# NVIDIA/nvalchemi-toolkit-ops

Measured on AMD Instinct MI355X. Metric: atom-steps/sec (nlist+D3+PME) on 100k-atom PBC box, higher is better.
Workload: dtype f64 (PME) + f32 (D3)

## Files before the change

### nvalchemi-toolkit-ops_amd/csrc/d3.hip

```cpp
#include <type_traits>
#include <mutex>

#include "common.h"
#include "binsort.h"

#ifdef MI_D3_IEEE
#define D3_RCP(x) (1.0f / (x))
#define D3_SQRT(x) sqrtf(x)
#else
#define D3_RCP(x) __builtin_amdgcn_rcpf(x)
#define D3_SQRT(x) __builtin_amdgcn_sqrtf(x)
#endif

namespace {

struct D3Dev {
  const float* rcov;
  const float* r4r2;
  const float4* tab;
  int nz;
  float a1, a2, s6, s8, k1, k3, s5_on, s5_off, inv_w;
  float4* crec;
  const float* crc;
  int* cflag;
// ... 17 lines not shown
  f.pad_code = S;
  return f;
}
__device__ __forceinline__ float d3_crec_encode(float d, int id, const D3CRec& f, bool* bad) {
  *bad = !(fabsf(d) < 256.0f);
  unsigned u = (unsigned)__float_as_int(d * f.down);
  if (f.mbit) u = (u + 1u) & ~1u;
  u |= ((unsigned)id << f.eshift) & f.emask;
  u |= ((unsigned)id >> f.eb) & f.mbit;
  return __int_as_float((int)u);
}
__device__ __forceinline__ int d3_crec_id(float w, const D3CRec& f) {
  const unsigned u = (unsigned)__float_as_int(w);
  return (int)(((u & f.emask) >> f.eshift) | ((u & f.mbit) << f.eb));
}
__device__ __forceinline__ float d3_crec_value(float w, const D3CRec& f) { return __int_as_float((int)((unsigned)__float_as_int(w) & f.clear)); }

struct D3Species;
__device__ __forceinline__ int d3_species_count(const D3Species* info);
struct D3ZeroSpec { const float* r0ab; float irs6, irs8, beta; };
struct D3ZeroPair { float i6, i8, bR; };
__device__ __forceinline__ D3ZeroPair d3_zero_pair(const D3ZeroSpec& Z, int zi, int zj, int nz) {
  const float R0 = Z.r0ab[(size_t)zi * nz + zj];
  const bool ok = R0 > 0.0f;
  D3ZeroPair p;
  p.i6 = ok ? Z.irs6 / R0 : 0.0f; p.i8 = ok ? Z.irs8 / R0 : 0.0f; p.bR = ok ? Z.beta * R0 : 0.0f;
  return p;
}
__device__ __forceinline__ float d3_zero_w(const D3ZeroSpec& Z, int zi, int zj, int nz, int pq) {
  if (Z.r0ab == nullptr || pq > 2) return 0.0f;
  const D3ZeroPair p = d3_zero_pair(Z, zi, zj, nz);
  return pq == 0 ? p.i6 : (pq == 1 ? p.i8 : p.bR);
}
struct D3Tables { const float* c6ab; const float* cnref; int nz; const D3Species* info; float4* tab; int first_block; D3ZeroSpec zero; };
__device__ __forceinline__ void d3_pack_tables_body(const float* __restrict__ c6ab, const float* __restrict__ cnref, int nz, const D3Species* __restrict__ info,
                                      float4* __restrict__ tab, long long vblock, const D3ZeroSpec& zero) {
  if (d3_species_count(info) <= 16) return;
  const long long t = vblock * blockDim.x + threadIdx.x;
  const long long total = (long long)nz * nz * 25;
  if (t >= total) return;
  const int pq = (int)(t % 25), p = pq / 5, q = pq % 5;
  const long long zz = t / 25;
  const int zj = (int)(zz % nz), zi = (int)(zz / nz);
  const float c6 = c6ab[t];
  const float ci = cnref[t];
  const float cj = cnref[(((long long)zj * nz + zi) * 5 + q) * 5 + p];
  tab[t] = make_float4(c6, ci, cj, d3_zero_w(zero, zi, zj, nz, pq));
}

template <class T> struct PairGeom { float r, rinv, rx, ry, rz; bool ok; };
struct Int3 { int a, b, c; };

#define D3_SORT_MIN_ATOMS 2048
#define D3_SORT_PER_BIN 16.0
template <class T> __device__ __forceinline__ T d3_code_pack(int place, int z);
template <> __device__ __forceinline__ float d3_code_pack<float>(int place, int z) { return __int_as_float((place << 7) | z); }
template <> __device__ __forceinline__ double d3_code_pack<double>(int place, int z) { return (double)(((long long)place << 7) | z); }
__device__ __forceinline__ int d3_code_of(float w) { return __float_as_int(w); }
__device__ __forceinline__ int d3_code_of(double w) { return (int)(long long)w; }

struct D3Grid { int cpd[3]; int off; };
template <class T>
__global__ void d3_sort_setup_kernel(const T* __restrict__ cell, int B, int N, float rc_est, D3Grid* __restrict__ grid, long long cap) {
  for (int s0 = 0; s0 < B; s0 += blockDim.x) {
    const int sidx = s0 + threadIdx.x;
    if (sidx < B) {
      T c[9], ci[9];
      for (int k = 0; k < 9; ++k) c[k] = cell[9 * (size_t)sidx + k];
      inverse3(c, ci);
      const double det = (double)c[0] * ((double)c[4] * c[8] - (double)c[5] * c[7]) - (double)c[1] * ((double)c[3] * c[8] - (double)c[5] * c[6]) +
// ... 39 lines not shown
    const int sidx = batch_idx ? batch_idx[i] : 0;
    const D3Grid G = grid[sidx];
    T c[9], ci[9];
    for (int k = 0; k < 9; ++k) c[k] = cell[9 * (size_t)sidx + k];
    inverse3(c, ci);
    const T x = pos[3 * (size_t)i], y = pos[3 * (size_t)i + 1], z = pos[3 * (size_t)i + 2];
    for (int d = 0; d < 3; ++d) {
      T f = x * ci[d] + y * ci[3 + d] + z * ci[6 + d];
      f = f - floor(f);
      const int q = (int)(f * (T)G.cpd[d]);
      n[d] = G.cpd[d];
      g[d] = q < 0 ? 0 : (q >= n[d] ? n[d] - 1 : q);
    }
    gs = sidx;
    key = G.off + (g[2] * n[1] + g[1]) * n[0] + g[0];
  }
  if (count) {
    if (in) keys[i] = key;
    bs_wave_add<false>(count, key, in);
  }
  const int nx_ = __shfl_down(g[0], 1, MI_WAVE), ny_ = __shfl_down(g[1], 1, MI_WAVE), nz_ = __shfl_down(g[2], 1, MI_WAVE), ns_ = __shfl_down(gs, 1, MI_WAVE);
  auto far = [](int a, int b, int m) { int d = a > b ? a - b : b - a; d = d < m - d ? d : m - d; return d > 1; };
  const bool pair = in && i + 1 < N && (threadIdx.x & (MI_WAVE - 1)) != MI_WAVE - 1;
  const bool bad = pair && (ns_ != gs || far(g[0], nx_, n[0]) || far(g[1], ny_, n[1]) || far(g[2], nz_, n[2]));
  const unsigned long long m = __ballot(bad);
  if (m && (threadIdx.x & (MI_WAVE - 1)) == 0) atomicAdd(incoherent, (int)__popcll(m));
}

#define D3_VERIFY_CHUNK 512
struct D3Guard {
  unsigned long long* slots; float K; const void* cell; int n_cell; const int* batch_idx;
  const int* nm; const int* nsh; const unsigned* words; const int* hdr_flag; int* flag; int M; int stride, phase; int atom_blocks;
};
template <class T>
__global__ void d3_pack_atoms_kernel(const T* __restrict__ pos, const int* __restrict__ numbers, int N, const float* __restrict__ rcov,
                                     const float* __restrict__ r4r2, const int* __restrict__ smap, int nz,
                                     typename Vec4<T>::type* __restrict__ apos, float4* __restrict__ aaux, float* __restrict__ forces,
                                     float* __restrict__ cn, float* __restrict__ dEdCN, float* __restrict__ e_atom, double* __restrict__ v_atom,
                                     const int* __restrict__ inv, typename Vec4<T>::type* __restrict__ apos_s, float4* __restrict__ aaux_s,
                                     typename Vec4<T>::type* __restrict__ acn, D3Guard G, D3Tables TB, float4* __restrict__ crec) {
  if ((int)blockIdx.x >= TB.first_block) {
    d3_pack_tables_body(TB.c6ab, TB.cnref, TB.nz, TB.info, TB.tab, (long long)blockIdx.x - TB.first_block, TB.zero);
    return;
  }
  if ((int)blockIdx.x >= G.atom_blocks) {
    const int lane = threadIdx.x & (MI_WAVE - 1);
    const int w = ((int)blockIdx.x - G.atom_blocks) * (blockDim.x / MI_WAVE) + threadIdx.x / MI_WAVE;
    if (w == 0 && lane == 0 && *G.hdr_flag != 0) *G.flag = 1;
    if (G.stride <= 0) return;
    const int chunks = 1, all_chunks = (G.M + D3_VERIFY_CHUNK - 1) / D3_VERIFY_CHUNK;
    const long long blk = w / chunks;
    const long long row = blk * G.stride + (long long)(((unsigned long long)G.phase + mi_mix64(0x51ull + (unsigned long long)blk)) % (unsigned long long)G.stride);
    if (row >= N) return;
    const int pick = G.stride == 1 ? -1 : (int)(mi_mix64(0x77ull + (unsigned long long)row * 1315423911ull + (unsigned long long)G.phase / (unsigned long long)G.stride) % (unsigned long long)all_chunks);
    const int t_beg = pick < 0 ? 0 : pick * D3_VERIFY_CHUNK, t_end = pick < 0 ? G.M : (t_beg + D3_VERIFY_CHUNK < G.M ? t_beg + D3_VERIFY_CHUNK : G.M);
    bool bad = false;
#pragma unroll 4
    for (int t = t_beg + lane; t < t_end; t += MI_WAVE) {
      const long long e = row * G.M + t;
      const int j = G.nm[e];
      const Int3 sh = reinterpret_cast<const Int3*>(G.nsh)[e];
      const unsigned cx = (unsigned)(sh.a + 1), cy = (unsigned)(sh.b + 1), cz = (unsigned)(sh.c + 1);
      const bool entry = (unsigned)j < (unsigned)N;
      const unsigned want = entry ? ((unsigned)j | ((cx & 3u) << 26) | ((cy & 3u) << 28) | (cz << 30)) : 0xffffffffu;
      bad |= G.words[e] != want || (entry && (cx > 2u || cy > 2u || cz > 2u));
    }
    if (bad) *G.flag = 1;
    return;
  }
  const int k = blockIdx.x * blockDim.x + threadIdx.x;
  if (G.slots) {
    unsigned long long h = 0;
    if (k < N) {
      const int a = inv ? inv[k] : k;
      h = mi_cn_atom_hash<T>(a, G.batch_idx ? G.batch_idx[a] : 0, pos[3 * (size_t)a], pos[3 * (size_t)a + 1], pos[3 * (size_t)a + 2],
                             mi_cn_rk(numbers[a], nz, rcov, G.K));
    }
    if (k < G.n_cell) h += mi_cn_cell_hash<T>(k, reinterpret_cast<const T*>(G.cell)[k]);
    if (k == 0) h += mi_cn_scale_hash(G.K);
    mi_cn_slot_add(G.slots, k / MI_WAVE, h);
  }
  if (k >= N) return;
  const int i = inv ? inv[k] : k;
  forces[3 * (size_t)i] = forces[3 * (size_t)i + 1] = forces[3 * (size_t)i + 2] = 0.0f;
  cn[i] = dEdCN[i] = e_atom[i] = 0.0f;
  if (v_atom)
    for (int k = 0; k < 9; ++k) v_atom[9 * (size_t)i + k] = 0.0;
  const int z = numbers[i];
  const bool real = z > 0 && z < nz;
  typename Vec4<T>::type r;
  r.x = pos[3 * (size_t)i]; r.y = pos[3 * (size_t)i + 1]; r.z = pos[3 * (size_t)i + 2];
  r.w = real ? (T)rcov[z] : (T)-1;
  apos[i] = r;
  const int sj = real ? smap[z] : -1;
  const float4 ax = make_float4(0.0f, real ? r4r2[z] : 0.0f, __int_as_float((z << 8) | (sj & 0xff)), 0.0f);
  aaux[i] = ax;
  if (crec) {
    const D3CRec f = d3_crec_format(d3_species_count(TB.info));
    bool bad;
    if (f.on) crec[k] = make_float4((float)r.x, (float)r.y, (float)r.z, d3_crec_encode(0.0f, sj >= 0 ? sj : f.pad_code, f, &bad));
  }
  if (inv) {
    apos_s[k] = r;
    aaux_s[k] = ax;
    r.w = d3_code_pack<T>(k, real ? z : 0);
    acn[i] = r;
  }
}

template <class T, class V4>
__device__ __forceinline__ PairGeom<T> d3_geom(const V4& pj, T pix, T piy, T piz, const Int3& sh, const T* __restrict__ cm, bool periodic) {
  PairGeom<T> g;
  T dx = pj.x - pix, dy = pj.y - piy, dz = pj.z - piz;
  if (periodic) {
    const T fs[3] = {(T)sh.a, (T)sh.b, (T)sh.c};
    T cart[3];
    const bool ortho = cm[1] == T(0) && cm[2] == T(0) && cm[3] == T(0) && cm[5] == T(0) && cm[6] == T(0) && cm[7] == T(0);
    if (ortho) { cart[0] = fs[0] * cm[0]; cart[1] = fs[1] * cm[4]; cart[2] = fs[2] * cm[8]; }
    else rowvec_mat3(fs, cm, cart);
    dx = dx + cart[0]; dy = dy + cart[1]; dz = dz + cart[2];
  }
  g.rx = (float)dx; g.ry = (float)dy; g.rz = (float)dz;
  const float r2 = g.rx * g.rx + g.ry * g.ry + g.rz * g.rz;
  g.ok = !(r2 < 1e-24f);
#ifdef MI_D3_IEEE
  g.r = sqrtf(g.ok ? r2 : 1.0f);
  const float rinv = 1.0f / g.r;
#else
  const float rinv = __builtin_amdgcn_rsqf(g.ok ? r2 : 1.0f);
  g.r = r2 * rinv;
#endif
// ... 232 lines not shown
    return;
  }
  const bool from_companion = *comp_flag == 0;
  for (int vb = blockIdx.x; vb < n_blocks; vb += gridDim.x) {
    if (from_companion) d3_cn_body<T, false, true, false, true>(D3_CN_ARGS, vb);
    else d3_cn_body<T, false, true, false, false>(D3_CN_ARGS, vb);
    __syncthreads();
  }
}
#undef D3_CN_ARGS
#undef D3_CN_PARAMS

__device__ __forceinline__ void d3_s5(float r, float on, float off, float inv_w, float& sw, float& dsw) {
  if (off <= on) { sw = 1.0f; dsw = 0.0f; return; }
  if (r <= on) { sw = 1.0f; dsw = 0.0f; return; }
  if (r >= off) { sw = 0.0f; dsw = 0.0f; return; }
  const float t = (r - on) * inv_w, t2 = t * t, t3 = t2 * t, t4 = t3 * t, t5 = t4 * t;
  sw = 1.0f - (10.0f * t3 - 15.0f * t4 + 6.0f * t5);
  dsw = (-30.0f * t2 + 60.0f * t3 - 30.0f * t4) * inv_w;
}

#define D3_SMAX 16

struct D3Species { int S; int factorized; int pad[2]; };
__device__ __forceinline__ int d3_species_count(const D3Species* info) { return info->S; }
#define D3_FROW 44

__global__ void d3_mark_species_kernel(const int* __restrict__ numbers, int N, int nz, int* __restrict__ present) {
  const int i = blockIdx.x * blockDim.x + threadIdx.x;
  if (i >= N) return;
  const int z = numbers[i];
  if (z > 0 && z < nz) present[z] = 1;
}
__global__ void d3_compact_species_kernel(const int* __restrict__ present, const float* __restrict__ c6ab, const float* __restrict__ cnref, int nz,
                                          int* __restrict__ smap, D3Species* __restrict__ info, float4* __restrict__ ctab,
                                          float* __restrict__ ftab, float* __restrict__ fcr, float k3, const float* __restrict__ r4r2,
                                          float a1, float a2, const float* __restrict__ rcov, float* __restrict__ crc, D3ZeroSpec zero) {
  __shared__ int zlist[D3_SMAX];
  __shared__ int count;
  __shared__ int fact_ok;
  if (threadIdx.x == 0) {
    fact_ok = 1;
    int S = 0;
    for (int z = 0; z < nz; ++z) {
      if (z > 0 && present[z]) { smap[z] = S < D3_SMAX ? S : -1; if (S < D3_SMAX) zlist[S] = z; ++S; }
      else smap[z] = -1;
    }
    count = S;
    info->S = S;
  }
  __syncthreads();
  const int S = count;
  if (S > D3_SMAX) { if (threadIdx.x == 0) info->factorized = 0; return; }
  if (threadIdx.x < 16) crc[threadIdx.x] = (int)threadIdx.x < S ? rcov[zlist[threadIdx.x]] : -1.0f;
  for (int k = threadIdx.x; k < S * S * 25; k += blockDim.x) {
    const int pq = k % 25, p = pq / 5, q = pq % 5, sj = (k / 25) % S, si = k / (25 * S);
    const int zi = zlist[si], zj = zlist[sj];
    const size_t a = ((size_t)zi * nz + zj) * 25 + pq, b = (((size_t)zj * nz + zi) * 5 + q) * 5 + p;
    ctab[k] = make_float4(c6ab[a], cnref[a], cnref[b], d3_zero_w(zero, zi, zj, nz, pq));
    ftab[((size_t)si * S + sj) * D3_FROW + p * 8 + q] = c6ab[a];
    const size_t dii = ((size_t)zi * nz + zi) * 25 + p * 6, djj = ((size_t)zj * nz + zj) * 25 + q * 6;
    const bool valid = c6ab[a] != 0.0f, rect = (c6ab[dii] != 0.0f) && (c6ab[djj] != 0.0f);
    const bool same = __float_as_int(cnref[a]) == __float_as_int(cnref[dii]) && __float_as_int(cnref[b]) == __float_as_int(cnref[djj]);
    if (valid != rect || (valid && !same)) fact_ok = 0;
  }
  for (int k = threadIdx.x; k < S * S * 5; k += blockDim.x) {
    float* row = ftab + (size_t)(k / 5) * D3_FROW + (k % 5) * 8;
    row[5] = row[6] = row[7] = 0.0f;
  }
  for (int k = threadIdx.x; k < S * S; k += blockDim.x) {
    const float q = 3.0f * r4r2[zlist[k / S]] * r4r2[zlist[k % S]];
    const float r0 = a1 * sqrtf(q) + a2, r02 = r0 * r0, r04 = r02 * r02;
    float* d = ftab + (size_t)k * D3_FROW + 40;
    if (zero.r0ab != nullptr) {
      const D3ZeroPair zp = d3_zero_pair(zero, zlist[k / S], zlist[k % S], nz);
      d[0] = q; d[1] = zp.i6; d[2] = zp.i8; d[3] = zp.bR;
      continue;
    }
    d[0] = q; d[1] = r04 * r02; d[2] = r04 * r04; d[3] = 0.0f;
  }
  for (int si = threadIdx.x; si < S; si += blockDim.x) {
    const int zi = zlist[si];
    int bits = 0;
    for (int p = 0; p < 5; ++p) {
      const size_t dii = ((size_t)zi * nz + zi) * 25 + p * 6;
      const bool has = c6ab[dii] != 0.0f;
      fcr[si * 8 + p] = has ? cnref[dii] : 1.0e30f;
      bits |= has << p;
    }
    fcr[si * 8 + 5] = __int_as_float(bits);
    fcr[si * 8 + 6] = fcr[si * 8 + 7] = 0.0f;
  }
  __syncthreads();
  if (threadIdx.x == 0) info->factorized = fact_ok && k3 < 0.0f;
}

__device__ __forceinline__ void d3_c6(float cn_i, float cn_j, const float4* __restrict__ t25, float k3, float& c6, float& dci) {
  float a[25];
  float mx = -1e20f, d0 = 0.0f;
#pragma unroll
  for (int c = 0; c < 5; ++c) {
    float4 v[5];
#pragma unroll
    for (int k = 0; k < 5; ++k) v[k] = t25[5 * c + k];
#pragma unroll
    for (int k = 0; k < 5; ++k) {
      const float di = cn_i - v[k].y, dj = cn_j - v[k].z;
      const float sq = di * di + dj * dj;
      const float at = (v[k].x != 0.0f) ? k3 * sq : -INFINITY;
      a[5 * c + k] = at;
      d0 = at > mx ? di : d0;
      mx = fmaxf(mx, at);
    }
    __builtin_amdgcn_sched_barrier(0);
  }
  float w = 0.0f, z = 0.0f, wdi = 0.0f, zdi = 0.0f;
#pragma unroll
  for (int t = 0; t < 25; ++t) {
    const float arg = a[t] - mx;
    const bool keep = !(arg < -12.0f);
    if (__builtin_amdgcn_ballot_w64(keep) == 0) continue;
    const float2 v = *reinterpret_cast<const float2*>(&t25[t]);
    const float di = (cn_i - v.y) - d0;
    const float L = keep ? d3_exp_neg(arg) : 0.0f;
    const float cL = v.x * L;
    w += L;
    z += cL;
// ... 513 lines not shown
      acc[k] = 0.0;
    }
  };
  for (int c = c0; c < c1; ++c) {
    const int i = c * MI_WAVE + lane;
    const bool in = i < N;
    const int s = in ? (batch_idx ? batch_idx[i] : 0) : -1;
    const int s0 = __shfl(s, 0, MI_WAVE);
    if (__all(!in || s == s0)) {
      if (s0 != cur) { flush(); cur = s0; }
      if (in) {
        acc[0] += (double)e_atom[i];
        if (want_virial) for (int k = 0; k < 9; ++k) acc[k + 1] += v_atom[9 * (size_t)i + k];
      }
    } else if (in) {
      atomicAdd(&sums[10 * ((size_t)s * D3_REDUCE_SLOTS + slot)], (double)e_atom[i]);
      if (want_virial) for (int k = 0; k < 9; ++k) atomicAdd(&sums[10 * ((size_t)s * D3_REDUCE_SLOTS + slot) + 1 + k], v_atom[9 * (size_t)i + k]);
    }
  }
  flush();
}
__global__ void d3_finish_kernel(const double* __restrict__ sums, int B, int want_virial, float* __restrict__ energy, float* __restrict__ virial) {
  const int t = blockIdx.x * blockDim.x + threadIdx.x;
  if (t >= 10 * B) return;
  const int s = t / 10, k = t - 10 * s;
  double v = 0.0;
#pragma unroll
  for (int q = 0; q < D3_REDUCE_SLOTS; ++q) v += sums[10 * ((size_t)s * D3_REDUCE_SLOTS + q) + k];
  if (k == 0) energy[s] = (float)v;
  else if (want_virial) virial[9 * (size_t)s + (k - 1)] = (float)v;
}

inline long long d3_sort_cap(int N, int B) { return 4ll * N + 8ll * (B > 0 ? B : 1); }
struct D3Layout { size_t dEdCN, e_atom, v_atom, guard, sums, tab, present, smap, sinfo, ctab, ftab, fcr, apos, aaux, aw, inv, skeys, sgrid, sbins, apos_s, acn, aaux_s, aw_s, dEdCN_s, crec, crc, total; };
D3Layout d3_layout(int N, int nz, int dtype, int B) {
  D3Layout L;
  size_t o = 0;
  auto take = [&](size_t b) { size_t at = o; o += mi_align(b); return at; };
  L.dEdCN = take(sizeof(float) * (size_t)N);
  L.e_atom = take(sizeof(float) * (size_t)N);
  L.v_atom = take(sizeof(double) * 9 * (size_t)N);
  L.guard = take(sizeof(unsigned long long) * MI_CN_SLOTS + 256);
  L.sums = take(sizeof(double) * 10 * D3_REDUCE_SLOTS * (size_t)(B > 0 ? B : 1));
  L.present = take(sizeof(int) * ((size_t)nz + 2));
  L.tab = take(sizeof(float4) * (size_t)nz * nz * 25);
  L.smap = take(sizeof(int) * (size_t)nz);
  L.sinfo = take(sizeof(D3Species));
  L.ctab = take(sizeof(float4) * D3_SMAX * D3_SMAX * 25);
  L.ftab = take(sizeof(float) * D3_SMAX * D3_SMAX * D3_FROW);
  L.fcr = take(sizeof(float) * D3_SMAX * 8);
  L.apos = take((dtype == MI_F32 ? 16 : 32) * (size_t)N);
  L.aaux = take(sizeof(float4) * (size_t)N);
  L.aw = take(sizeof(float4) * 2 * (size_t)N);
  L.inv = take(sizeof(int) * (size_t)N);
  L.skeys = take(sizeof(int) * (size_t)N);
  L.sgrid = take(sizeof(D3Grid) * (size_t)(B > 0 ? B : 1));
  L.sbins = take(sizeof(int) * bs_scratch_ints(d3_sort_cap(N, B) + 1));
  L.apos_s = take((dtype == MI_F32 ? 16 : 32) * (size_t)N);
  L.acn = take((dtype == MI_F32 ? 16 : 32) * (size_t)N);
  L.aaux_s = take(sizeof(float4) * (size_t)N);
  L.aw_s = take(sizeof(float4) * 2 * (size_t)N);
  L.dEdCN_s = take(sizeof(float) * (size_t)N);
  L.crec = take(sizeof(float4) * (size_t)N);
  L.crc = take(sizeof(float) * 16);
  L.total = o;
  return L;
}

#define D3_ORDER_PROBE_EVERY 64
#define D3_ORDER_SLOTS 8
struct D3OrderState { int* h_count = nullptr;  int n_atoms = -1, n_systems = -1; long long calls = 0; unsigned gen = 0; };
static D3OrderState g_d3_order[16];
static std::mutex g_d3_order_mu;
static bool d3_order_decide(int N, int B, hipStream_t st, bool* probe, float* rc_est, int** publish_to) {
  *probe = false;
  *publish_to = nullptr;
  *rc_est = 0.0f;
  const char* force = getenv("NVALCHEMIOPS_D3_SORT");
  if (force && atoi(force) == 0) return false;
  int dev = 0;
  if (hipGetDevice(&dev) != hipSuccess || dev < 0 || dev >= 16) return false;
  hipStreamCaptureStatus cap = hipStreamCaptureStatusNone;
  const bool capturing = hipStreamIsCapturing(st, &cap) == hipSuccess && cap != hipStreamCaptureStatusNone;
  std::lock_guard<std::mutex> lock(g_d3_order_mu);
  D3OrderState& S = g_d3_order[dev];
  if (!S.h_count) {
    if (capturing || hipHostMalloc(reinterpret_cast<void**>(&S.h_count), 2 * D3_ORDER_SLOTS * sizeof(int), hipHostMallocDefault) != hipSuccess) { S.h_count = nullptr; return force != nullptr; }
    for (int k = 0; k < 2 * D3_ORDER_SLOTS; ++k) S.h_count[k] = 0;
  }
  if (S.n_atoms != N || S.n_systems != B) {
    S.n_atoms = N; S.n_systems = B; S.calls = 0; ++S.gen;
    S.h_count[2 * (S.gen % D3_ORDER_SLOTS)] = 0; S.h_count[2 * (S.gen % D3_ORDER_SLOTS) + 1] = 0;
  }
  volatile int* h = S.h_count + 2 * (S.gen % D3_ORDER_SLOTS);
  *publish_to = S.h_count + 2 * (S.gen % D3_ORDER_SLOTS);
  *probe = !capturing && (S.calls < 4 || (S.calls % D3_ORDER_PROBE_EVERY) == 0);
  ++S.calls;
// ... 33 lines not shown
  float4* aw = reinterpret_cast<float4*>(ws + L.aw);
  const bool sortable = pk != nullptr && cell != nullptr && N >= D3_SORT_MIN_ATOMS && N < (1 << 24) && hp->nz <= 128;
  int* order_probe = present + hp->nz;
  bool probe = false;
  float rc_est = 0.0f;
  int* order_slot = nullptr;
  const bool sorted = sortable && d3_order_decide(N, B, st, &probe, &rc_est, &order_slot);
  if (pre && !sorted) {
    pk = const_cast<unsigned*>(pre_words);
    pk_flag = gflag;
  } else if (ws_pk_flag) {
    MI_HIP_CHECK(hipMemsetAsync(ws_pk_flag, 0, sizeof(int), st));
  }
  int* inv = sorted ? reinterpret_cast<int*>(ws + L.inv) : nullptr;
  auto* apos_s = reinterpret_cast<typename Vec4<T>::type*>(ws + L.apos_s);
  auto* acn = reinterpret_cast<typename Vec4<T>::type*>(ws + L.acn);
  float4* aaux_s = reinterpret_cast<float4*>(ws + L.aaux_s);
  float4* aw_s = reinterpret_cast<float4*>(ws + L.aw_s);
  float* dEdCN_s = reinterpret_cast<float*>(ws + L.dEdCN_s);
  D3Dev P;
  P.rcov = hp->rcov; P.r4r2 = hp->r4r2; P.tab = tab; P.nz = hp->nz;
  P.a1 = hp->a1; P.a2 = hp->a2; P.s6 = hp->s6; P.s8 = hp->s8; P.k1 = hp->k1; P.k3 = hp->k3; P.s5_on = hp->s5_on; P.s5_off = hp->s5_off;
  D3ZeroSpec zero{nullptr, 0.0f, 0.0f, 0.0f};
  if constexpr (DAMP == D3_DAMP_ZERO) {
    P.a1 = zp->alpha; P.a2 = 0.0f;
    zero = D3ZeroSpec{zp->r0ab, 1.0f / zp->rs6, 1.0f / zp->rs8, zp->beta};
  }
  P.inv_w = (hp->s5_off > hp->s5_on) ? (float)(1.0 / ((double)hp->s5_off - (double)hp->s5_on)) : 0.0f;
  const char* crec_env = getenv("NVALCHEMIOPS_D3_CHAIN_RECORDS");
  const bool crec_off = crec_env && crec_env[0] == '0';
  P.crec = (sizeof(T) == 4 && !crec_off) ? reinterpret_cast<float4*>(ws + L.crec) : nullptr;
  P.crc = reinterpret_cast<const float*>(ws + L.crc);
  P.cflag = gflag + 4;
  MI_HIP_CHECK(hipMemsetAsync(ws + L.guard, 0, ((L.present - L.guard) + sizeof(int) * ((size_t)hp->nz + 2) + 15) / 16 * 16, st));
  D3Grid* sgrid = reinterpret_cast<D3Grid*>(ws + L.sgrid);
  if (sorted || (sortable && probe)) {
    d3_sort_setup_kernel<T><<<1, 256, 0, st>>>(cell, B, N, rc_est, sgrid, d3_sort_cap(N, B));
    MI_LAUNCH_CHECK();
  }
  if (sorted) {
    int* skeys = reinterpret_cast<int*>(ws + L.skeys);
    const BsScratch bins = bs_carve(reinterpret_cast<int*>(ws + L.sbins), d3_sort_cap(N, B) + 1);
    MI_HIP_CHECK(bs_clear(bins, st));
    d3_sort_key_kernel<T><<<mi_blocks(N, 256), 256, 0, st>>>(pos, cell, batch_idx, N, sgrid, skeys, bins.count, order_probe);
    MI_LAUNCH_CHECK();
    MI_HIP_CHECK(bs_sort(bins, skeys, N, nullptr, inv, nullptr, st));
  } else if (sortable && probe) {
    d3_sort_key_kernel<T><<<mi_blocks(N, 256), 256, 0, st>>>(pos, cell, batch_idx, N, sgrid, nullptr, nullptr, order_probe);
    MI_LAUNCH_CHECK();
  }
  const bool publish = sortable && probe;
  d3_mark_species_kernel<<<mi_blocks(N, 256), 256, 0, st>>>(numbers, N, hp->nz, present);
  MI_LAUNCH_CHECK();
  d3_compact_species_kernel<<<1, 256, 0, st>>>(present, hp->c6ab, hp->cn_ref, hp->nz, smap, sinfo, ctab, ftab, fcr, hp->k3, hp->r4r2, hp->a1, hp->a2, hp->rcov,
                                               reinterpret_cast<float*>(ws + L.crc), zero);
  MI_LAUNCH_CHECK();
  const long long nt = (long long)hp->nz * hp->nz * 25;
  const bool use_cn = !CSR && cn_block != nullptr && pre != nullptr && !sorted;
  D3Guard G{};
  G.atom_blocks = mi_blocks(use_cn && 9 * B > N ? 9 * B : N, 256);
  int verify_blocks = 0;
  if (use_cn) { G.slots = gslots; G.K = mi_cn_scale(hp->k1); G.cell = cell; G.n_cell = 9 * B; G.batch_idx = batch_idx; }
  if (pre) {
    G.nm = idx; G.nsh = ush; G.words = pre_words; G.hdr_flag = pre_flag; G.flag = gflag; G.M = M; G.stride = verify_stride; G.phase = verify_phase;
    verify_blocks = verify_stride > 0 ? mi_blocks(((long long)N + verify_stride - 1) / verify_stride, 4) : 1;
  }
  const D3Tables TB{hp->c6ab, hp->cn_ref, hp->nz, sinfo, tab, G.atom_blocks + verify_blocks, zero};
  d3_pack_atoms_kernel<T><<<G.atom_blocks + verify_blocks + mi_blocks(nt, 256), 256, 0, st>>>(pos, numbers, N, hp->rcov, hp->r4r2, smap, hp->nz, apos, aaux, forces, cn,
                                                                                              dEdCN, e_atom, want_virial ? v_atom : nullptr, inv, apos_s, aaux_s, acn, G, TB, P.crec);
  MI_LAUNCH_CHECK();
  const int blocks = mi_blocks(N, 4);
  const D3Weights W{sinfo, fcr, hp->k3, sizeof(T) == 4 ? reinterpret_cast<const float4*>(apos) : nullptr, aw, aw_s};
#define MI_D3_CN(BIG_, SORT_, PKIN_, OUT_, OUTFLAG_, GATE_, WANT_)                                                                                 \
  d3_cn_kernel<T, CSR, BIG_, SORT_, PKIN_><<<mi_blocks(N, D3_LS_WAVES), D3_LS_WAVES * MI_WAVE, 0, st>>>(                                             \
      pos, numbers, N, idx, ush, nptr, M, fill_value, cell, batch_idx, P, apos, aaux, cn, OUT_, OUTFLAG_, inv, acn, aaux_s,                           \
      sortable ? order_probe + 1 : nullptr, pre_words, W, GATE_, WANT_)
  const bool big_list = (double)n_entries * ((cell && ush) ? 16.0 : 4.0) > 2.0e9;
  if constexpr (!CSR) {
    if (use_cn) {
      const int n_blocks = mi_blocks(N, D3_LS_WAVES);
      const int* hdr = reinterpret_cast<const int*>(cn_block);
      MI_TIMED("d3_cn", st, (d3_cn_pre_kernel<T><<<n_blocks < D3_CN_PRE_GRID ? n_blocks : D3_CN_PRE_GRID, D3_LS_WAVES * MI_WAVE, 0, st>>>(
                                pos, numbers, N, idx, ush, nptr, M, fill_value, cell, batch_idx, P, apos, aaux, cn, nullptr, nullptr, inv, acn, aaux_s,
                                sortable ? order_probe + 1 : nullptr, pre_words, W, gflag, hdr, gslots,
                                reinterpret_cast<const float*>((const char*)cn_block + MI_CN_HEADER_BYTES), n_blocks)));
    } else if (pre) {
      unsigned* out = sorted ? pk : nullptr;
      int* outflag = sorted ? pk_flag : nullptr;
      if (sorted) { MI_TIMED("d3_cn", st, (MI_D3_CN(true, true, true, out, outflag, gflag, 0))); MI_D3_CN(true, true, false, out, outflag, gflag, 1); }
      else { MI_TIMED("d3_cn", st, (MI_D3_CN(true, false, true, out, outflag, gflag, 0))); MI_D3_CN(true, false, false, out, outflag, gflag, 1); }
    }
  }
  if (!pre) {
    if (big_list) { if (sorted) { MI_TIMED("d3_cn", st, (MI_D3_CN(true, true, false, pk, pk_flag, nullptr, 0))); } else { MI_TIMED("d3_cn", st, (MI_D3_CN(true, false, false, pk, pk_flag, nullptr, 0))); } }
    else { if (sorted) { MI_TIMED("d3_cn", st, (MI_D3_CN(false, true, false, pk, pk_flag, nullptr, 0))); } else { MI_TIMED("d3_cn", st, (MI_D3_CN(false, false, false, pk, pk_flag, nullptr, 0))); } }
  }
#undef MI_D3_CN
  if (publish) d3_order_publish(order_probe, order_slot, st);
  MI_LAUNCH_CHECK();
  auto launch_energy = [&](auto mode, auto packed) {
    constexpr int MODE_ = decltype(mode)::value;
    constexpr bool PK_ = decltype(packed)::value;
// ... 219 lines not shown
```

### nvalchemi-toolkit-ops_amd/csrc/d3_atm.h

```cpp
#pragma once
#include "atm_core.h"

#define D3_ATM_TILE 320
#define D3_ATM_REC 13
#define D3_ATM_LDS_S 6
#define D3_ATM_E12 6.14421235e-06f

struct D3AtmMath { static __device__ __forceinline__ float rcp(float x) { return D3_RCP(x); } };

template <int MODE>
__device__ __forceinline__ float d3_atm_c6_jk(const float (*tp)[D3_ATM_TILE], int p, const float (*tq)[D3_ATM_TILE], int q, int S, int nz,
                                              const float* ft, const float4* __restrict__ t25base, float k3) {
  const int cp = __float_as_int(tp[ATM_CODE][p]), cq = __float_as_int(tq[ATM_CODE][q]);
  if constexpr (MODE == 2) {
    const float* rows = ft + (size_t)(cp * S + cq) * D3_FROW;
    float w = 0.0f, z = 0.0f;
#pragma unroll
    for (int a = 0; a < 5; ++a) {
      const float va = tp[ATM_TAIL + a][p];
      if (__builtin_amdgcn_readfirstlane(__float_as_int(va)) == 0) continue;
#pragma unroll
      for (int b = 0; b < 5; ++b) {
        float L = va * tq[ATM_TAIL + b][q];
        L = L >= D3_ATM_E12 ? L : 0.0f;
// ... 178 lines not shown
  D3Species* sinfo = reinterpret_cast<D3Species*>(ws + L.sinfo);
  float4* ctab = reinterpret_cast<float4*>(ws + L.ctab);
  float* ftab = reinterpret_cast<float*>(ws + L.ftab);
  float* fcr = reinterpret_cast<float*>(ws + L.fcr);
  auto* apos = reinterpret_cast<typename Vec4<T>::type*>(ws + L.apos);
  auto* apos_s = reinterpret_cast<typename Vec4<T>::type*>(ws + L.apos_s);
  auto* acn = reinterpret_cast<typename Vec4<T>::type*>(ws + L.acn);
  float4* aaux = reinterpret_cast<float4*>(ws + L.aaux);
  float4* aaux_s = reinterpret_cast<float4*>(ws + L.aaux_s);
  float4* aw = reinterpret_cast<float4*>(ws + L.aw);
  float4* aw_s = reinterpret_cast<float4*>(ws + L.aw_s);
  float* dEdCN_s = reinterpret_cast<float*>(ws + L.dEdCN_s);
  float* cn = reinterpret_cast<float*>(ws + LA.cn);
  D3Dev P;
  P.rcov = hp->rcov; P.r4r2 = hp->r4r2; P.tab = tab; P.nz = hp->nz;
  P.a1 = hp->a1; P.a2 = hp->a2; P.s6 = hp->s6; P.s8 = hp->s8; P.k1 = hp->k1; P.k3 = hp->k3; P.s5_on = hp->s5_on; P.s5_off = hp->s5_off;
  P.inv_w = 0.0f;
  const D3ZeroSpec zero = DAMP == D3_DAMP_ZERO ? D3ZeroSpec{r0ab, 1.0f, 1.0f, rs9} : D3ZeroSpec{nullptr, 0.0f, 0.0f, 0.0f};
  P.crec = nullptr;
  P.crc = reinterpret_cast<const float*>(ws + L.crc);
  P.cflag = gflag + 4;
  MI_HIP_CHECK(hipMemsetAsync(ws + L.guard, 0, ((L.present - L.guard) + sizeof(int) * ((size_t)hp->nz + 2) + 15) / 16 * 16, st));
  MI_HIP_CHECK(hipMemsetAsync(ws + LA.visits, 0, sizeof(unsigned) * (size_t)N, st));
  d3_mark_species_kernel<<<mi_blocks(N, 256), 256, 0, st>>>(numbers, N, hp->nz, present);
  MI_LAUNCH_CHECK();
  d3_compact_species_kernel<<<1, 256, 0, st>>>(present, hp->c6ab, hp->cn_ref, hp->nz, smap, sinfo, ctab, ftab, fcr, hp->k3, hp->r4r2, hp->a1, hp->a2, hp->rcov,
                                               reinterpret_cast<float*>(ws + L.crc), zero);
  MI_LAUNCH_CHECK();
  const long long nt = (long long)hp->nz * hp->nz * 25;
  D3Guard G{};
  G.atom_blocks = mi_blocks(N, 256);
  const D3Tables TB{hp->c6ab, hp->cn_ref, hp->nz, sinfo, tab, G.atom_blocks, zero};
  d3_pack_atoms_kernel<T><<<G.atom_blocks + mi_blocks(nt, 256), 256, 0, st>>>(pos, numbers, N, hp->rcov, hp->r4r2, smap, hp->nz, apos, aaux, forces, cn, dEdCN, e_atom,
                                                                            want_virial ? v_atom : nullptr, nullptr, apos_s, aaux_s, acn, G, TB, nullptr);
  MI_LAUNCH_CHECK();
  const D3Weights W{sinfo, fcr, hp->k3, nullptr, aw, aw_s};
  MI_TIMED("d3_atm_cn", st, (d3_cn_kernel<T, CSR, false, false, false><<<mi_blocks(N, D3_LS_WAVES), D3_LS_WAVES * MI_WAVE, 0, st>>>(
                                pos, numbers, N, idx, ush, nptr, M, fill_value, cell, batch_idx, P, apos, aaux, cn, nullptr, nullptr, nullptr, acn, aaux_s, nullptr,
                                nullptr, W, nullptr, 0)));
  MI_LAUNCH_CHECK();
  const AtmParams A{s9, alpha, cutoff * cutoff, reinterpret_cast<unsigned*>(ws + LA.visits)};
  auto launch = [&](auto mode) {
    constexpr int MODE_ = decltype(mode)::value;
    d3_atm_kernel<T, CSR, MODE_, DAMP><<<N, ATM_WAVES * MI_WAVE, 0, st>>>(pos, numbers, N, idx, ush, nptr, M, fill_value, cell, batch_idx, P, A, cn, want_virial, smap,
                                                                    sinfo, ctab, ftab, fcr, apos, aaux, aw, dEdCN, forces, e_atom, v_atom);
  };
  MI_TIMED("d3_atm_triples", st, (launch(std::integral_constant<int, 2>{}), launch(std::integral_constant<int, 1>{}), launch(std::integral_constant<int, 0>{})));
  MI_LAUNCH_CHECK();
  MI_TIMED("d3_atm_chain", st, (d3_chain_kernel<T, CSR, false><<<mi_blocks(N, D3_CH_LS_WAVES), D3_CH_LS_WAVES * MI_WAVE, 0, st>>>(
                                   pos, numbers, N, idx, ush, nptr, M, fill_value, cell, batch_idx, P, apos, dEdCN, want_virial, forces, v_atom, nullptr, nullptr,
                                   nullptr, apos_s, dEdCN_s, sinfo)));
  MI_LAUNCH_CHECK();
  double* sums = reinterpret_cast<double*>(ws + L.sums);
  d3_reduce_kernel<<<D3_REDUCE_WAVES / 4, 256, 0, st>>>(e_atom, v_atom, batch_idx, N, want_virial, sums);
  MI_LAUNCH_CHECK();
  d3_finish_kernel<<<mi_blocks(10ll * B, 256), 256, 0, st>>>(sums, B, want_virial, energy, virial);
  MI_LAUNCH_CHECK();
  return MI_OK;
}
```

Before: 31.54 million.

## Fuse D3 species marking and compaction into clear and pack-atoms kernels

Replaces the workspace memset, the species-mark kernel and the single-block compact kernel with one clear+mark kernel that builds per-block species bitmasks. The pack-atoms kernel then gets an extra block that runs compaction from the OR-reduced mask. Atom blocks derive compact species ids from the mask rank instead of reading smap. This removes two launches and a serial dependency from the D3 prelude. In exchange every pack block re-gathers up to 256 mask entries, and correctness relies on the rank matching the compaction order for up to 16 species.

```diff
diff --git a/nvalchemi-toolkit-ops_amd/csrc/d3.hip b/nvalchemi-toolkit-ops_amd/csrc/d3.hip
--- a/nvalchemi-toolkit-ops_amd/csrc/d3.hip
+++ b/nvalchemi-toolkit-ops_amd/csrc/d3.hip
@@ -73,10 +73,72 @@
   const D3ZeroPair p = d3_zero_pair(Z, zi, zj, nz);
   return pq == 0 ? p.i6 : (pq == 1 ? p.i8 : p.bR);
 }
+#define D3_MARK_GRID 256
+#define D3_MASK_MAX_NZ 128
+struct D3Mask { unsigned w[4]; };
+__device__ __forceinline__ int d3_mask_rank(const D3Mask& m, int z) {
+  int r = 0;
+#pragma unroll
+  for (int k = 0; k < 4; ++k) {
+    const int lo = z - 32 * k;
+    const unsigned below = lo >= 32 ? 0xffffffffu : (lo > 0 ? ((1u << lo) - 1u) : 0u);
+    r += __popc(m.w[k] & below);
+  }
+  return r;
+}
+__device__ __forceinline__ int d3_mask_count(const D3Mask& m) { return __popc(m.w[0]) + __popc(m.w[1]) + __popc(m.w[2]) + __popc(m.w[3]); }
+__device__ __forceinline__ bool d3_mask_has(const D3Mask& m, int z) {
+  const unsigned w = z < 32 ? m.w[0] : (z < 64 ? m.w[1] : (z < 96 ? m.w[2] : m.w[3]));
+  return z >= 0 && z < D3_MASK_MAX_NZ && ((w >> (z & 31)) & 1u) != 0u;
+}
+__device__ __forceinline__ D3Mask d3_mask_block_or(D3Mask m) {
+  __shared__ unsigned acc[4];
+  if (threadIdx.x < 4) acc[threadIdx.x] = 0u;
+  __syncthreads();
+#pragma unroll
+  for (int k = 0; k < 4; ++k) {
+    unsigned v = m.w[k];
+#pragma unroll
+    for (int o = MI_WAVE / 2; o > 0; o >>= 1) v |= (unsigned)__shfl_xor((int)v, o, MI_WAVE);
+    if ((threadIdx.x & (MI_WAVE - 1)) == 0 && v != 0u) atomicOr(&acc[k], v);
+  }
+  __syncthreads();
+  D3Mask r;
+#pragma unroll
+  for (int k = 0; k < 4; ++k) r.w[k] = acc[k];
+  return r;
+}
+__device__ __forceinline__ D3Mask d3_mask_gather(const uint4* __restrict__ marks, int n_marks) {
+  D3Mask m{{0u, 0u, 0u, 0u}};
+  for (int t = threadIdx.x; t < n_marks; t += blockDim.x) {
+    const uint4 v = marks[t];
+    m.w[0] |= v.x; m.w[1] |= v.y; m.w[2] |= v.z; m.w[3] |= v.w;
+  }
+  return d3_mask_block_or(m);
+}
+__global__ __launch_bounds__(256) void d3_clear_mark_kernel(const int* __restrict__ numbers, int N, int nz, uint4* __restrict__ marks, int n_marks,
+                                                            uint4* __restrict__ zero, long long n_zero) {
+  if ((int)blockIdx.x >= n_marks) {
+    const long long stride = (long long)(gridDim.x - n_marks) * blockDim.x;
+    for (long long q = (long long)((int)blockIdx.x - n_marks) * blockDim.x + threadIdx.x; q < n_zero; q += stride) zero[q] = make_uint4(0u, 0u, 0u, 0u);
+    return;
+  }
+  D3Mask m{{0u, 0u, 0u, 0u}};
+  for (long long i = (long long)blockIdx.x * blockDim.x + threadIdx.x; i < N; i += (long long)n_marks * blockDim.x) {
+    const int z = numbers[i];
+    if (z > 0 && z < nz) {
+#pragma unroll
+      for (int k = 0; k < 4; ++k) m.w[k] |= (z >> 5) == k ? (1u << (z & 31)) : 0u;
+    }
+  }
+  m = d3_mask_block_or(m);
+  if (threadIdx.x == 0) marks[blockIdx.x] = make_uint4(m.w[0], m.w[1], m.w[2], m.w[3]);
+}
+
 struct D3Tables { const float* c6ab; const float* cnref; int nz; const D3Species* info; float4* tab; int first_block; D3ZeroSpec zero; };
-__device__ __forceinline__ void d3_pack_tables_body(const float* __restrict__ c6ab, const float* __restrict__ cnref, int nz, const D3Species* __restrict__ info,
+__device__ __forceinline__ void d3_pack_tables_body(const float* __restrict__ c6ab, const float* __restrict__ cnref, int nz, int n_species,
                                       float4* __restrict__ tab, long long vblock, const D3ZeroSpec& zero) {
-  if (d3_species_count(info) <= 16) return;
+  if (n_species <= 16) return;
   const long long t = vblock * blockDim.x + threadIdx.x;
   const long long total = (long long)nz * nz * 25;
   if (t >= total) return;
@@ -182,20 +244,37 @@
   unsigned long long* slots; float K; const void* cell; int n_cell; const int* batch_idx;
   const int* nm; const int* nsh; const unsigned* words; const int* hdr_flag; int* flag; int M; int stride, phase; int atom_blocks;
 };
+struct D3Fused {
+  const uint4* marks; int n_marks;
+  const float* r4r2; int* smap; D3Species* info; float4* ctab; float* ftab; float* fcr; float* crc; float k3, a1, a2;
+};
+__device__ void d3_compact_body(const int* __restrict__ present, const D3Mask& mask, const float* __restrict__ c6ab, const float* __restrict__ cnref, int nz,
+                                int* __restrict__ smap, D3Species* __restrict__ info, float4* __restrict__ ctab, float* __restrict__ ftab,
+                                float* __restrict__ fcr, float k3, const float* __restrict__ r4r2, float a1, float a2, const float* __restrict__ rcov,
+                                float* __restrict__ crc, const D3ZeroSpec& zero);
 template <class T>
 __global__ void d3_pack_atoms_kernel(const T* __restrict__ pos, const int* __restrict__ numbers, int N, const float* __restrict__ rcov,
                                      const float* __restrict__ r4r2, const int* __restrict__ smap, int nz,
                                      typename Vec4<T>::type* __restrict__ apos, float4* __restrict__ aaux, float* __restrict__ forces,
                                      float* __restrict__ cn, float* __restrict__ dEdCN, float* __restrict__ e_atom, double* __restrict__ v_atom,
                                      const int* __restrict__ inv, typename Vec4<T>::type* __restrict__ apos_s, float4* __restrict__ aaux_s,
-                                     typename Vec4<T>::type* __restrict__ acn, D3Guard G, D3Tables TB, float4* __restrict__ crec) {
-  if ((int)blockIdx.x >= TB.first_block) {
-    d3_pack_tables_body(TB.c6ab, TB.cnref, TB.nz, TB.info, TB.tab, (long long)blockIdx.x - TB.first_block, TB.zero);
+                                     typename Vec4<T>::type* __restrict__ acn, D3Guard G, D3Tables TB, float4* __restrict__ crec, D3Fused F) {
+  const bool fused = F.marks != nullptr;
+  const int bid = (int)blockIdx.x - (fused ? 1 : 0);
+  const bool check_block = bid >= G.atom_blocks && bid < TB.first_block;
+  D3Mask mask{{0u, 0u, 0u, 0u}};
+  if (fused && !check_block) mask = d3_mask_gather(F.marks, F.n_marks);
+  if (bid < 0) {
+    d3_compact_body(nullptr, mask, TB.c6ab, TB.cnref, TB.nz, F.smap, F.info, F.ctab, F.ftab, F.fcr, F.k3, F.r4r2, F.a1, F.a2, rcov, F.crc, TB.zero);
     return;
   }
-  if ((int)blockIdx.x >= G.atom_blocks) {
+  if (bid >= TB.first_block) {
+    d3_pack_tables_body(TB.c6ab, TB.cnref, TB.nz, fused ? d3_mask_count(mask) : d3_species_count(TB.info), TB.tab, (long long)bid - TB.first_block, TB.zero);
+    return;
+  }
+  if (check_block) {
     const int lane = threadIdx.x & (MI_WAVE - 1);
-    const int w = ((int)blockIdx.x - G.atom_blocks) * (blockDim.x / MI_WAVE) + threadIdx.x / MI_WAVE;
+    const int w = (bid - G.atom_blocks) * (blockDim.x / MI_WAVE) + threadIdx.x / MI_WAVE;
     if (w == 0 && lane == 0 && *G.hdr_flag != 0) *G.flag = 1;
     if (G.stride <= 0) return;
     const int chunks = 1, all_chunks = (G.M + D3_VERIFY_CHUNK - 1) / D3_VERIFY_CHUNK;
@@ -218,7 +297,7 @@
     if (bad) *G.flag = 1;
     return;
   }
-  const int k = blockIdx.x * blockDim.x + threadIdx.x;
+  const int k = bid * blockDim.x + threadIdx.x;
   if (G.slots) {
     unsigned long long h = 0;
     if (k < N) {
@@ -242,11 +321,15 @@
   r.x = pos[3 * (size_t)i]; r.y = pos[3 * (size_t)i + 1]; r.z = pos[3 * (size_t)i + 2];
   r.w = real ? (T)rcov[z] : (T)-1;
   apos[i] = r;
-  const int sj = real ? smap[z] : -1;
+  int sj = -1;
+  if (real) {
+    if (fused) { const int rank = d3_mask_rank(mask, z); sj = rank < 16 ? rank : -1; }
+    else sj = smap[z];
+  }
   const float4 ax = make_float4(0.0f, real ? r4r2[z] : 0.0f, __int_as_float((z << 8) | (sj & 0xff)), 0.0f);
   aaux[i] = ax;
   if (crec) {
-    const D3CRec f = d3_crec_format(d3_species_count(TB.info));
+    const D3CRec f = d3_crec_format(fused ? d3_mask_count(mask) : d3_species_count(TB.info));
     bool bad;
     if (f.on) crec[k] = make_float4((float)r.x, (float)r.y, (float)r.z, d3_crec_encode(0.0f, sj >= 0 ? sj : f.pad_code, f, &bad));
   }
@@ -545,10 +628,11 @@
   const int z = numbers[i];
   if (z > 0 && z < nz) present[z] = 1;
 }
-__global__ void d3_compact_species_kernel(const int* __restrict__ present, const float* __restrict__ c6ab, const float* __restrict__ cnref, int nz,
-                                          int* __restrict__ smap, D3Species* __restrict__ info, float4* __restrict__ ctab,
-                                          float* __restrict__ ftab, float* __restrict__ fcr, float k3, const float* __restrict__ r4r2,
-                                          float a1, float a2, const float* __restrict__ rcov, float* __restrict__ crc, D3ZeroSpec zero) {
+static_assert(D3_SMAX == 16, "d3_pack_atoms_kernel derives compact ids below 16 from the species mask");
+__device__ void d3_compact_body(const int* __restrict__ present, const D3Mask& mask, const float* __restrict__ c6ab, const float* __restrict__ cnref, int nz,
+                                int* __restrict__ smap, D3Species* __restrict__ info, float4* __restrict__ ctab, float* __restrict__ ftab,
+                                float* __restrict__ fcr, float k3, const float* __restrict__ r4r2, float a1, float a2, const float* __restrict__ rcov,
+                                float* __restrict__ crc, const D3ZeroSpec& zero) {
   __shared__ int zlist[D3_SMAX];
   __shared__ int count;
   __shared__ int fact_ok;
@@ -556,7 +640,7 @@
     fact_ok = 1;
     int S = 0;
     for (int z = 0; z < nz; ++z) {
-      if (z > 0 && present[z]) { smap[z] = S < D3_SMAX ? S : -1; if (S < D3_SMAX) zlist[S] = z; ++S; }
+      if (z > 0 && (present ? present[z] != 0 : d3_mask_has(mask, z))) { smap[z] = S < D3_SMAX ? S : -1; if (S < D3_SMAX) zlist[S] = z; ++S; }
       else smap[z] = -1;
     }
     count = S;
@@ -606,6 +690,12 @@
   }
   __syncthreads();
   if (threadIdx.x == 0) info->factorized = fact_ok && k3 < 0.0f;
+}
+__global__ void d3_compact_species_kernel(const int* __restrict__ present, const float* __restrict__ c6ab, const float* __restrict__ cnref, int nz,
+                                          int* __restrict__ smap, D3Species* __restrict__ info, float4* __restrict__ ctab,
+                                          float* __restrict__ ftab, float* __restrict__ fcr, float k3, const float* __restrict__ r4r2,
+                                          float a1, float a2, const float* __restrict__ rcov, float* __restrict__ crc, D3ZeroSpec zero) {
+  d3_compact_body(present, D3Mask{{0u, 0u, 0u, 0u}}, c6ab, cnref, nz, smap, info, ctab, ftab, fcr, k3, r4r2, a1, a2, rcov, crc, zero);
 }
 
 __device__ __forceinline__ void d3_c6(float cn_i, float cn_j, const float4* __restrict__ t25, float k3, float& c6, float& dci) {
@@ -1185,7 +1275,7 @@
 }
 
 inline long long d3_sort_cap(int N, int B) { return 4ll * N + 8ll * (B > 0 ? B : 1); }
-struct D3Layout { size_t dEdCN, e_atom, v_atom, guard, sums, tab, present, smap, sinfo, ctab, ftab, fcr, apos, aaux, aw, inv, skeys, sgrid, sbins, apos_s, acn, aaux_s, aw_s, dEdCN_s, crec, crc, total; };
+struct D3Layout { size_t dEdCN, e_atom, v_atom, guard, sums, tab, present, smap, sinfo, ctab, ftab, fcr, apos, aaux, aw, inv, skeys, sgrid, sbins, apos_s, acn, aaux_s, aw_s, dEdCN_s, crec, crc, marks, total; };
 D3Layout d3_layout(int N, int nz, int dtype, int B) {
   D3Layout L;
   size_t o = 0;
@@ -1216,6 +1306,7 @@
   L.dEdCN_s = take(sizeof(float) * (size_t)N);
   L.crec = take(sizeof(float4) * (size_t)N);
   L.crc = take(sizeof(float) * 16);
+  L.marks = take(sizeof(uint4) * D3_MARK_GRID);
   L.total = o;
   return L;
 }
@@ -1315,7 +1406,19 @@
   P.crec = (sizeof(T) == 4 && !crec_off) ? reinterpret_cast<float4*>(ws + L.crec) : nullptr;
   P.crc = reinterpret_cast<const float*>(ws + L.crc);
   P.cflag = gflag + 4;
-  MI_HIP_CHECK(hipMemsetAsync(ws + L.guard, 0, ((L.present - L.guard) + sizeof(int) * ((size_t)hp->nz + 2) + 15) / 16 * 16, st));
+  const size_t clear_bytes = ((L.present - L.guard) + sizeof(int) * ((size_t)hp->nz + 2) + 15) / 16 * 16;
+  const char* prelude_env = getenv("NVALCHEMIOPS_D3_PRELUDE");
+  const bool fused = hp->nz <= D3_MASK_MAX_NZ && !(prelude_env && prelude_env[0] == '0');
+  uint4* marks = reinterpret_cast<uint4*>(ws + L.marks);
+  const int n_marks = mi_blocks(N, 256) < D3_MARK_GRID ? mi_blocks(N, 256) : D3_MARK_GRID;
+  if (fused) {
+    const long long n_zero = (long long)(clear_bytes / 16);
+    const int zero_blocks = mi_blocks(n_zero, 256) < 64 ? mi_blocks(n_zero, 256) : 64;
+    d3_clear_mark_kernel<<<n_marks + zero_blocks, 256, 0, st>>>(numbers, N, hp->nz, marks, n_marks, reinterpret_cast<uint4*>(ws + L.guard), n_zero);
+    MI_LAUNCH_CHECK();
+  } else {
+    MI_HIP_CHECK(hipMemsetAsync(ws + L.guard, 0, clear_bytes, st));
+  }
   D3Grid* sgrid = reinterpret_cast<D3Grid*>(ws + L.sgrid);
   if (sorted || (sortable && probe)) {
     d3_sort_setup_kernel<T><<<1, 256, 0, st>>>(cell, B, N, rc_est, sgrid, d3_sort_cap(N, B));
@@ -1333,11 +1436,14 @@
     MI_LAUNCH_CHECK();
   }
   const bool publish = sortable && probe;
-  d3_mark_species_kernel<<<mi_blocks(N, 256), 256, 0, st>>>(numbers, N, hp->nz, present);
-  MI_LAUNCH_CHECK();
-  d3_compact_species_kernel<<<1, 256, 0, st>>>(present, hp->c6ab, hp->cn_ref, hp->nz, smap, sinfo, ctab, ftab, fcr, hp->k3, hp->r4r2, hp->a1, hp->a2, hp->rcov,
-                                               reinterpret_cast<float*>(ws + L.crc), zero);
-  MI_LAUNCH_CHECK();
+  if (!fused) {
+    d3_mark_species_kernel<<<mi_blocks(N, 256), 256, 0, st>>>(numbers, N, hp->nz, present);
+    MI_LAUNCH_CHECK();
+    d3_compact_species_kernel<<<1, 256, 0, st>>>(present, hp->c6ab, hp->cn_ref, hp->nz, smap, sinfo, ctab, ftab, fcr, hp->k3, hp->r4r2, hp->a1, hp->a2, hp->rcov,
+                                                 reinterpret_cast<float*>(ws + L.crc), zero);
+    MI_LAUNCH_CHECK();
+  }
+  const D3Fused F{fused ? marks : nullptr, n_marks, hp->r4r2, smap, sinfo, ctab, ftab, fcr, reinterpret_cast<float*>(ws + L.crc), hp->k3, hp->a1, hp->a2};
   const long long nt = (long long)hp->nz * hp->nz * 25;
   const bool use_cn = !CSR && cn_block != nullptr && pre != nullptr && !sorted;
   D3Guard G{};
@@ -1349,8 +1455,8 @@
     verify_blocks = verify_stride > 0 ? mi_blocks(((long long)N + verify_stride - 1) / verify_stride, 4) : 1;
   }
   const D3Tables TB{hp->c6ab, hp->cn_ref, hp->nz, sinfo, tab, G.atom_blocks + verify_blocks, zero};
-  d3_pack_atoms_kernel<T><<<G.atom_blocks + verify_blocks + mi_blocks(nt, 256), 256, 0, st>>>(pos, numbers, N, hp->rcov, hp->r4r2, smap, hp->nz, apos, aaux, forces, cn,
-                                                                                              dEdCN, e_atom, want_virial ? v_atom : nullptr, inv, apos_s, aaux_s, acn, G, TB, P.crec);
+  d3_pack_atoms_kernel<T><<<(fused ? 1 : 0) + G.atom_blocks + verify_blocks + mi_blocks(nt, 256), 256, 0, st>>>(pos, numbers, N, hp->rcov, hp->r4r2, smap, hp->nz, apos, aaux, forces, cn,
+                                                                                              dEdCN, e_atom, want_virial ? v_atom : nullptr, inv, apos_s, aaux_s, acn, G, TB, P.crec, F);
   MI_LAUNCH_CHECK();
   const int blocks = mi_blocks(N, 4);
   const D3Weights W{sinfo, fcr, hp->k3, sizeof(T) == 4 ? reinterpret_cast<const float4*>(apos) : nullptr, aw, aw_s};
diff --git a/nvalchemi-toolkit-ops_amd/csrc/d3_atm.h b/nvalchemi-toolkit-ops_amd/csrc/d3_atm.h
--- a/nvalchemi-toolkit-ops_amd/csrc/d3_atm.h
+++ b/nvalchemi-toolkit-ops_amd/csrc/d3_atm.h
@@ -234,7 +234,7 @@
   G.atom_blocks = mi_blocks(N, 256);
   const D3Tables TB{hp->c6ab, hp->cn_ref, hp->nz, sinfo, tab, G.atom_blocks, zero};
   d3_pack_atoms_kernel<T><<<G.atom_blocks + mi_blocks(nt, 256), 256, 0, st>>>(pos, numbers, N, hp->rcov, hp->r4r2, smap, hp->nz, apos, aaux, forces, cn, dEdCN, e_atom,
-                                                                            want_virial ? v_atom : nullptr, nullptr, apos_s, aaux_s, acn, G, TB, nullptr);
+                                                                            want_virial ? v_atom : nullptr, nullptr, apos_s, aaux_s, acn, G, TB, nullptr, D3Fused{});
   MI_LAUNCH_CHECK();
   const D3Weights W{sinfo, fcr, hp->k3, nullptr, aw, aw_s};
   MI_TIMED("d3_atm_cn", st, (d3_cn_kernel<T, CSR, false, false, false><<<mi_blocks(N, D3_LS_WAVES), D3_LS_WAVES * MI_WAVE, 0, st>>>(
```

After: 31.59 million, median of 2. Within noise of the previous version (+0.2%).
